# LANL-Bioinformatics/PCRamp

Measured on AMD Instinct MI355X. Metric: primer-pair x target amplification evals/sec, higher is better.
Workload: dtype u32

## Files before the change

pcramp_amd/csrc/pcr_device.hip:

```cpp
#include <hip/hip_runtime.h>
#include <cstring>
#include <rocprim/device/device_radix_sort.hpp>

#include <stdint.h>
#include <string.h>
#include <math.h>
#include <stdlib.h>
#include <string>
#include <vector>
#include <chrono>
#include <algorithm>
#include <unordered_map>
#include <type_traits>
#include <thread>
#include <mutex>
#include <condition_variable>
#include <functional>
#include <memory>
#include <atomic>
#include <cassert>
#include <sched.h>
#include <pthread.h>

#include "../../include/pcramp_hip.h"
// ... 133 lines not shown
		cgh = hi.y | hi.z;
	}
	uint32_t out = 0;
	for(uint32_t j = 0;j < 32;++j){
		if(funnel(nzl, nzh, j) != 0xFFFFFFFFu) continue;
		const uint32_t ngc = __popc(funnel(cgl, cgh, j));
		if(!((gc_ok >> ngc) & 1ull)) continue;
		const uint32_t n2 = __popc(funnel(d2l, d2h, j));
		const uint32_t n3 = __popc(funnel(d3l, d3h, j));
		const uint32_t n4 = __popc(funnel(d4l, d4h, j));
		const uint32_t e = n2 + 2*n4;
		bool exceeds;
		if(e >= 33){ exceeds = true; }
		else{
			uint64_t p3 = 1;
			for(uint32_t k = 0;k < n3;++k) p3 *= 3;
			exceeds = p3 > ((uint64_t)max_degen >> e);
		}
		if(!exceeds) out |= (1u << j);
	}
	valid[gb] = out;
}

struct HitSink { uint32_t *best; Hit *hits; uint32_t *seq_count; uint32_t *counters; uint32_t cap; uint32_t ncand; uint32_t epoch; };

__device__ __forceinline__ void record_hit_inline(const HitSink &k, uint32_t seq, uint32_t cand, uint64_t key, uint32_t cnt)
{
	const uint32_t tagged = (k.epoch << 8) | cnt;
	const uint32_t old = atomicMax(&k.best[(size_t)seq*k.ncand + cand], tagged);
	if(tagged >= old){
		const uint32_t slot = atomicAdd(&k.seq_count[seq], 1u);
		if(slot < k.cap){
			Hit h; h.key = key; h.cand = cand; h.cnt = cnt;
			k.hits[(size_t)seq*k.cap + slot] = h;
		}
		else{ atomicOr(&k.counters[0], 1u); atomicMax(&k.counters[2], slot + 1); }
	}
}

__device__ __noinline__ void record_hit(const HitSink k, uint32_t seq, uint32_t cand, uint64_t key, uint32_t cnt)
{
	record_hit_inline(k, seq, cand, key, cnt);
}

__device__ __forceinline__ uint64_t make_key(uint32_t seq, int32_t loc, uint32_t strand , uint32_t kind, uint32_t ord)
{
	return ((uint64_t)seq << KEY_SEQ_SHIFT) | ((uint64_t)(uint32_t)(loc + LOC_BIAS) << KEY_LOC_SHIFT) |
// ... 411 lines not shown
	Stream stream;
	Stream aux_stream;
	std::string design_text;
	DevBuf<uint64_t> split_where;
	pcr_params params;
	pcrhost::PackFilter filt;
	SeqSet sets[PCR_N_SETS];
	DevBuf<uint32_t> best, counters, mask, status;
	int scan_version = 3;
	bool force_seed1 = false;
	struct S2Key { uint32_t a, c, g, t, floor_; bool operator==(const S2Key &o) const { return a == o.a && c == o.c && g == o.g && t == o.t && floor_ == o.floor_; } };
	struct S2KeyHash { size_t operator()(const S2Key &k) const { uint64_t h = 0x9E3779B97F4A7C15ull; for(uint32_t v : {k.a, k.c, k.g, k.t, k.floor_}){ h ^= v; h *= 0x100000001B3ull; h ^= h >> 29; } return (size_t)h; } };
	struct S2Entry { std::vector<uint32_t> seeds;  uint32_t off_mask; bool seedable; uint4 mask;  };
	std::unordered_map<S2Key, S2Entry, S2KeyHash> s2_cache;
	std::vector<pcrhost::Seed> s2_tmp;
	static constexpr int S3_CHUNK_SETS = 4;
	struct S3Chunks { uint64_t gen = 0; uint32_t total = 0; std::vector<uint32_t> run; };
	struct S3Entry : S2Entry { std::vector<uint8_t> spans;  S3Chunks chunks[S3_CHUNK_SETS]; uint32_t next_slot = 0; };
	std::unordered_map<S2Key, S3Entry, S2KeyHash> s3_cache;
	std::vector<pcrhost::FoldSeed> s3_tmp;
	struct S3Launch { Seed3Slices W; uint32_t n_chunks, per_wg, slice_cap, n_irr_wg; };
	bool no_seed3 = false, s3_attr_set = false;
	bool s3_next = true;
	bool s2_attr_set = false; uint32_t s2_dbg = 0; bool no_irr_index = false;
	std::unordered_map<S2Key, S2Entry, S2KeyHash> s1_cache;
	DevBuf<uint32_t> s1_image, s1_heads, s1_multi, s1_part;
	bool host_seed_tables = false;
	DevBuf<Hit> hits;
	DevBuf<uint64_t> bits_fr, bits_rf;
	DevBuf<OligoDev> oligos;
	DevBuf<SwJob> sw_jobs; DevBuf<SwOut> sw_out; DevBuf<uint8_t> sw_q, sw_qlen, sw_t, entry_codes, entry_lens;
	DevBuf<AmpRec> amp_recs, amp_recs2; DevBuf<BgPairDev> bg_pairs;
	DevBuf<uint64_t> amp_keys; DevBuf<uint32_t> amp_pkeys, amp_pair_start; DevBuf<uint8_t> sort_tmp;
	DevBuf<thermo::Job> th_jobs; DevBuf<thermo::JobOut> th_out; DevBuf<int> th_dg; DevBuf<uint2> th_map; DevBuf<uint32_t> th_bad;
	float th_dg_salt = -1.0f;
	DevBuf<unsigned long long> th_dbg; bool th_attr_set = false;
	std::vector<thermo::Job> th_host_jobs; std::vector<thermo::JobOut> th_host_res;
	MappedBuf<uint8_t> sw_pin; Event sw_done[2];
	DevBuf<pcr_amplicon> mx_amp;
	DevBuf<OligoDev> opt_oligos; DevBuf<uint2> opt_jobs; DevBuf<float> opt_cov; DevBuf<uint32_t> opt_loc, opt_tasks;
	DevBuf<Planes> mx_keys; uint32_t mx_n_keys = 0; DevBuf<uint32_t> mx_count;
	DevBuf<uint8_t> pool_in, pool_tmp; DevBuf<uint32_t> pool_cnt, pool_ord; DevBuf<uint64_t> pool_eoff, pool_ioff, pool_keys; DevBuf<uint2> pool_items; DevBuf<pcr_product> pool_rec;
	DevBuf<uint8_t> site_in, site_tmp; DevBuf<uint32_t> site_cnt, site_ord, site_flag; DevBuf<uint64_t> site_eoff, site_joff, site_keys; DevBuf<uint2> site_items; DevBuf<float4> site_res; DevBuf<pcr_site> site_rec;
	bool site_attr_set = false;
	pcr_comm *shard_comm = nullptr; uint64_t shard_first = 0, shard_n_total = 0; int shard_mode = 0;
	DevBuf<uint64_t> sh_rec, sh_full; DevBuf<uint8_t> sh_stage;
	std::vector<uint64_t> shard_bounds; DevBuf<uint64_t> d_shard_bounds;
	bool design_ready = false; DevBuf<uint64_t> sh_bits;
	std::vector<std::vector<uint8_t> > samp_packed; std::vector<uint64_t> samp_len;
	void drop_shard(){ shard_comm = nullptr; shard_mode = 0; shard_bounds.clear(); design_ready = false; samp_packed.clear(); samp_len.clear(); }
	pcr_comm *trial_comm = nullptr;
// ... 619 lines not shown
	if(hipGetDeviceProperties(&prop, device) != hipSuccess){ g_err = "pcr_create: hipGetDeviceProperties failed"; return nullptr; }
	if(std::string(prop.gcnArchName).find("gfx950") == std::string::npos){
		g_err = std::string("pcr_create: device is ") + prop.gcnArchName + ", this build targets gfx950 only";
		return nullptr;
	}
	pcr_ctx *ctx = new pcr_ctx();
	ctx->device = device;
	if(hip_stream) ctx->stream.borrow((hipStream_t)hip_stream);
	else if(ctx->stream.create() != hipSuccess){ g_err = "pcr_create: hipStreamCreate failed"; delete ctx; return nullptr; }
	if(params){ ctx->params = *params; }
	else{ ctx->params.pack_max_degen = 256; ctx->params.pack_min_gc = 0.0f; ctx->params.pack_max_gc = 1.0f; }
	{ hipDeviceProp_t prop; if(hipGetDeviceProperties(&prop, device) == hipSuccess && prop.multiProcessorCount > 0) ctx->n_cu = (uint32_t)prop.multiProcessorCount; }
	if(const char *v = getenv("PCRAMP_TIMING")) ctx->timing = v[0] == '1';
	ctx->debug_log = getenv("PCRAMP_DEBUG") != nullptr;
	if(const char *v = getenv("PCRAMP_DEBUG_EPOCH")) ctx->debug_epoch = (uint32_t)strtoul(v, nullptr, 0);
	if(const char *v = getenv("PCRAMP_OPT_PM")) ctx->opt_pm_global = v[0] == 'g';
	if(const char *v = getenv("PCRAMP_DEBUG_OPT_TASKS")){ unsigned a = 0, b = 0; if(sscanf(v, "%u,%u", &a, &b) >= 1){ ctx->opt_dbg_wg_tasks = a; ctx->opt_dbg_task_cap = b; } }
	if(const char *v = getenv("PCRAMP_SEED")) ctx->force_seed1 = v[0] == '1';
	if(const char *v = getenv("PCRAMP_SEED_TABLES")) ctx->host_seed_tables = v[0] == 'h';
	if(const char *v = getenv("PCRAMP_S2DBG")) ctx->s2_dbg = (uint32_t)atoi(v);
	if(const char *v = getenv("PCRAMP_IRR_INDEX")) ctx->no_irr_index = v[0] == '0';
	if(const char *v = getenv("PCRAMP_SEED3")) ctx->no_seed3 = v[0] == '0';
	if(const char *v = getenv("PCRAMP_S3_NEXT")) ctx->s3_next = v[0] != '0';
	if(const char *v = getenv("PCRAMP_LAUNCH_THREAD")) ctx->launch_thread = v[0] != '0';
	if(const char *v = getenv("PCRAMP_SCAN")){ if(v[0] == '1') ctx->scan_version = 1; else if(v[0] == '2') ctx->scan_version = 2; }
	{
		const char *v = getenv("PCRAMP_STAGE");
		if(!(v && v[0] == 'k') && prop.isLargeBar){
			DevBuf<uint32_t> probe(true); MappedBuf<uint32_t> back; const std::string err_before = g_err;
			constexpr uint32_t PROBE_WORDS = 1024;
			if(probe.ensure(PROBE_WORDS) == PCR_OK && back.ensure(PROBE_WORDS*sizeof(uint32_t)) == PCR_OK){
				hipPointerAttribute_t at;
				bool ok = hipPointerGetAttributes(&at, probe.p) == hipSuccess;
				for(int round = 0;ok && round < 2;++round){
					volatile uint32_t *w = (volatile uint32_t *)probe.p;
					for(uint32_t i = 0;i < PROBE_WORDS;++i){ w[i] = 0x9E3779B9u*(i + 1) + (uint32_t)round; back.host[i] = 0; }
					__builtin_ia32_sfence();
					hipLaunchKernelGGL(k_stage, dim3(1), dim3(256), 0, ctx->stream, (const uint4 *)probe.p, (uint4 *)back.dev, PROBE_WORDS/4,
						(uint4 *)nullptr, 0u, (uint4 *)nullptr, 0u, (uint4 *)nullptr, 0u);
					ok = hipGetLastError() == hipSuccess && hipStreamSynchronize(ctx->stream) == hipSuccess;
					for(uint32_t i = 0;ok && i < PROBE_WORDS;++i) ok = back.host[i] == 0x9E3779B9u*(i + 1) + (uint32_t)round;
				}
				ctx->direct_ok = ok;
			}
			else{ (void)hipGetLastError(); g_err = err_before; }
		}
// ... 624 lines not shown
```

pcramp_amd/csrc/pcr_host.hpp:

```cpp
#ifndef PCR_HOST_HPP
#define PCR_HOST_HPP

#include <stdint.h>
#include <algorithm>
#include <deque>
#include <vector>

namespace pcrhost {

struct Planes {
	uint32_t a, c, g, t;
};

inline uint32_t bitrev32(uint32_t v)
{
	v = ((v >> 1) & 0x55555555u) | ((v & 0x55555555u) << 1);
	v = ((v >> 2) & 0x33333333u) | ((v & 0x33333333u) << 2);
	v = ((v >> 4) & 0x0F0F0F0Fu) | ((v & 0x0F0F0F0Fu) << 4);
	v = ((v >> 8) & 0x00FF00FFu) | ((v & 0x00FF00FFu) << 8);
	return (v >> 16) | (v << 16);
}

inline unsigned word_get(const uint64_t w[2], int k) { return (unsigned)(w[k >> 4] >> ((15 - (k & 15))*4)) & 0xF; }

// ... 24 lines not shown
	p.c = gather_every_4th(r[0] >> 1) | (gather_every_4th(r[1] >> 1) << 16);
	p.g = gather_every_4th(r[0] >> 2) | (gather_every_4th(r[1] >> 2) << 16);
	p.t = gather_every_4th(r[0] >> 3) | (gather_every_4th(r[1] >> 3) << 16);
	return p;
}

inline void word_of_planes(const Planes &p, uint64_t w[2])
{
	w[0] = w[1] = 0;
	for(int k = 0;k < 32;++k){
		const unsigned v = ((p.a >> k) & 1) | (((p.c >> k) & 1) << 1) | (((p.g >> k) & 1) << 2) | (((p.t >> k) & 1) << 3);
		word_set(w, k, v);
	}
}

inline Planes planes_revcomp(const Planes &p)
{
	Planes r;
	r.a = bitrev32(p.t);
	r.t = bitrev32(p.a);
	r.c = bitrev32(p.g);
	r.g = bitrev32(p.c);
	return r;
}

inline uint32_t planes_occupied(const Planes &p) { return p.a | p.c | p.g | p.t; }
inline int planes_size(const Planes &p) { return __builtin_popcount(planes_occupied(p)); }
inline int planes_start(const Planes &p) { const uint32_t o = planes_occupied(p); return o ? __builtin_ctz(o) : 32; }
inline int planes_stop(const Planes &p) { const uint32_t o = planes_occupied(p); return o ? 31 - __builtin_clz(o) : -1; }

inline unsigned planes_nibble(const Planes &p, int k)
{
	return ((p.a >> k) & 1) | (((p.c >> k) & 1) << 1) | (((p.g >> k) & 1) << 2) | (((p.t >> k) & 1) << 3);
}

inline Planes planes_shift_left(const Planes &p) { Planes r = {p.a >> 1, p.c >> 1, p.g >> 1, p.t >> 1}; return r; }
inline Planes planes_shift_right(const Planes &p) { Planes r = {p.a << 1, p.c << 1, p.g << 1, p.t << 1}; return r; }

struct PackFilter {
	uint32_t max_degen;
	uint64_t gc_ok;
	bool gc_on;

	void set_gc(float min_gc, float max_gc)
	{
		gc_on = (min_gc > 0.0f) || (max_gc < 1.0f);
// ... 658 lines not shown
```

pcramp_amd/csrc/pcr_scan_seed3.inc:

```

constexpr uint32_t PIX_CODES = 1u << 18;
constexpr uint32_t PIX_KEYS = PIX_CODES << 2;
constexpr uint32_t S3_BATCH = 8;

template<bool SCATTER>
__global__ void k_pix_build(const uint32_t *__restrict__ tb, const uint32_t *__restrict__ blk_seq, const uint64_t *__restrict__ blk_off,
	const uint64_t *__restrict__ len, uint64_t total_blocks, uint32_t *__restrict__ count_or_cursor, uint4 *__restrict__ ent)
{
	const uint64_t b = (uint64_t)blockIdx.x*blockDim.x + threadIdx.x;
	if(b >= total_blocks) return;
	const uint32_t seq = blk_seq[b];
	const int64_t p0 = (int64_t)(b - blk_off[seq])*32, L = (int64_t)len[seq];
	uint32_t w[8];
#pragma unroll
	for(int k = 0;k < 8;++k) w[k] = tb[(int64_t)2*(int64_t)b - 2 + k];
#pragma unroll
	for(int i = 0;i < 32;++i){
		if(p0 + i + 9 > L) break;
		const uint32_t ten = (i < 16) ? funnel(w[2], w[3], 2*i) : funnel(w[3], w[4], 2*(i - 16));
		const uint32_t code = ((ten & S2_CODE_MASK) << 2) | ((ten >> 18) & 3u);
		if(SCATTER){
			const uint32_t at = atomicAdd(&count_or_cursor[code], 1u);
			const int jl = (i + 9) >> 4, sl = 2*((i + 9) & 15);
			const int jr = (i + 41) >> 4, sr = 2*((i + 41) & 15);
// ... 53 lines not shown
		const uint32_t sdv = (lane < 16u && i < T3.n_seeds) ? T3.seeds[i] : S2_END;
		const uint32_t orient = T3.or_base + (sdv & 0x1FFu);
		uint32_t first = 0, cnt = 0;
		if(sdv != S2_END && !(orient & 1u)){
			const uint32_t key = (((sdv >> 9) & 31u) << 18) | (sdv >> 14);
			first = IA.ix_first[key]; cnt = IA.ix_last[key] - first;
		}
		const uint32_t incl = s2_scan(cnt);
		const uint32_t total = s2_rl(incl, 63);
		for(uint32_t t0 = 0;t0 < total;t0 += 64u){
			const uint32_t t = t0 + lane;
			uint32_t lo = 0;
#pragma unroll
			for(uint32_t stp = 32u;stp;stp >>= 1){ if((uint32_t)__shfl((int)incl, (int)(lo + stp - 1u)) <= t) lo += stp; }
			const int sl = (int)min(lo, 63u);
			const uint32_t s_incl = (uint32_t)__shfl((int)incl, sl), s_cnt = (uint32_t)__shfl((int)cnt, sl), s_first = (uint32_t)__shfl((int)first, sl);
			const uint32_t c = (uint32_t)__shfl((int)orient, sl) >> 1;
			if(t >= total) continue;
			const IrrDev e = IA.irr[IA.ix_words[s_first + (t - (s_incl - s_cnt))]];
			if(((e.meta >> 8) & 0xFFu) < IA.min_cws || !Q.active[e.seq]) continue;
			const uint32_t n = match_count(e.w.a, e.w.c, e.w.g, e.w.t, cand_fwd[c]);
			if(n >= cand_floor[c]) record_hit(sink, e.seq, c, make_key(e.seq, e.loc, e.meta & 0xFF, 1, (e.meta >> 16) & 0xFF), n);
		}
	}
}

template<uint32_t S3_THREADS>
__global__ __launch_bounds__(S3_THREADS) __attribute__((amdgpu_waves_per_eu(8, 8))) void k_seed3(Seed3Tables T3, Seed3Set Q, IrrArgs2 IA, const uint4 *__restrict__ cand_fwd, const uint32_t *__restrict__ cand_floor,
	HitSink sink, S2Clear Z, Seed3Slices W)
{
	extern __shared__ uint4 s3_dyn[];
	uint4 *const masks = s3_dyn;
	uint32_t *const prefix = (uint32_t *)(masks + T3.n_or);
	uint32_t *const seeds = prefix + T3.slice_cap;
	uint8_t *const floors = (uint8_t *)(seeds + T3.slice_cap);
	uint8_t *const spans = floors + ((T3.n_or + 15u) & ~15u);
	const uint32_t wave = threadIdx.x >> 6, lane = threadIdx.x & 63u;
	for(uint32_t i = blockIdx.x*S3_THREADS + threadIdx.x;i < Z.n0;i += gridDim.x*S3_THREADS) Z.z0[i] = make_uint4(0, 0, 0, 0);
	for(uint32_t i = blockIdx.x*S3_THREADS + threadIdx.x;i < Z.n1;i += gridDim.x*S3_THREADS) Z.z1[i] = make_uint4(0, 0, 0, 0);
	if(Z.ctrl && blockIdx.x == 0 && threadIdx.x == 0){ Z.ctrl[1] = 0; Z.ctrl[3] = 0; }
	for(uint32_t i = threadIdx.x;i < T3.n_or;i += S3_THREADS){ masks[i] = T3.masks[i]; floors[i] = T3.floors[i]; }
	constexpr uint32_t S3_WAVES = S3_THREADS/64;
	if(blockIdx.x < T3.n_irr_wg){
		if(IA.ix_first) s3_irregular(T3, Q, IA, cand_fwd, cand_floor, sink, blockIdx.x*S3_WAVES + wave, T3.n_irr_wg*S3_WAVES, lane);
		return;
	}
// ... 10 lines not shown
			const uint32_t q = q0 + lane*S3_WAVES;
			if(lane < S3_BATCH && q < q_hi){
				uint32_t lo = 0, hi = n_slice - 1u;
				while(hi - lo > 1u){ const uint32_t mid = (lo + hi) >> 1; if(prefix[mid] <= q) lo = mid; else hi = mid; }
				c_sd = seeds[lo];
				const uint32_t key = (c_sd >> 14) << 2, sp = spans[lo];
				const uint32_t f = T3.pix_first[key + (sp & 3u)], e = T3.pix_last[key + (sp >> 2)], j0 = (q - prefix[lo])*64u;
				c_first = f + j0; c_cnt = (e - f) - j0;
			}
		}
		uint4 en[S3_BATCH];
#pragma unroll
		for(int b = 0;b < (int)S3_BATCH;++b){
			const uint32_t first = s2_rl(c_first, b), cnt = s2_rl(c_cnt, b);
			en[b] = make_uint4(0xFFFFFFFFu, 0, 0, 0);
			if(lane < cnt) en[b] = T3.pix_ent[first + lane];
		}
		uint32_t cnt_b[S3_BATCH], g[S3_BATCH]; bool pass_b[S3_BATCH];
#pragma unroll
		for(int b = 0;b < (int)S3_BATCH;++b){
			const uint32_t sdv = s2_rl(c_sd, b);
			const uint32_t off = (sdv >> 9) & 31u, local = sdv & 0x1FFu, code = sdv >> 14;
			g[b] = en[b].x;
			const uint32_t r_lo = funnel(en[b].z, en[b].w, 14);
			const uint4 cx = make_uint4(en[b].y << 2, (funnel(en[b].y, en[b].z, 30) & 0xFFFFu) | (code << 16), (code >> 16) | (r_lo << 2), en[b].w >> 12);
			const uint32_t in = 24u - off, sh = 2u*(in & 15u);
			const uint32_t a0 = (in < 16u) ? funnel(cx.x, cx.y, sh) : funnel(cx.y, cx.z, sh);
			const uint32_t a1 = (in < 16u) ? funnel(cx.y, cx.z, sh) : funnel(cx.z, cx.w, sh);
			cnt_b[b] = (uint32_t)__popc(s2_mux(a0, a1, masks[local]));
			pass_b[b] = g[b] != 0xFFFFFFFFu && cnt_b[b] >= floors[local] && g[b] >= off;
		}
		uint32_t vw[S3_BATCH], info[S3_BATCH], bl[S3_BATCH];
#pragma unroll
		for(int b = 0;b < (int)S3_BATCH;++b){
			vw[b] = 0; info[b] = 0; bl[b] = 0;
			if(pass_b[b]){
				const uint32_t ws = g[b] - ((s2_rl(c_sd, b) >> 9) & 31u);
				vw[b] = Q.valid[ws >> 5]; info[b] = Q.blk_info[ws >> 5]; bl[b] = Q.blk_local[ws >> 5];
			}
		}
#pragma unroll
		for(int b = 0;b < (int)S3_BATCH;++b){
			if(!pass_b[b]) continue;
			const uint32_t sdv = s2_rl(c_sd, b);
			const uint32_t ws = g[b] - ((sdv >> 9) & 31u), seq = info[b] & BLK_SEQ_MASK;
			if(!((vw[b] >> (ws & 31u)) & 1u) || (info[b] & (BLK_DEGEN | BLK_INACTIVE))) continue;
			const uint32_t p_local = bl[b]*32u + (ws & 31u);
			const uint32_t orient = T3.or_base + (sdv & 0x1FFu), c = orient >> 1;
			if(orient & 1u) record_hit(sink, seq, c, make_key(seq, (int32_t)p_local + 31, 2, 0, 0), cnt_b[b]);
			else record_hit(sink, seq, c, make_key(seq, (int32_t)p_local, 1, 0, 0), cnt_b[b]);
		}
	}
	if(IA.ix_first && T3.n_irr_wg == 0) s3_irregular(T3, Q, IA, cand_fwd, cand_floor, sink, gw, n_gw, lane);
}
```

pcramp_amd/csrc/pcr_screen.inc:

```
__device__ __forceinline__ bool db_slot(uint32_t g, uint32_t n, uint32_t cap, const uint32_t *__restrict__ touched,
	const uint32_t *__restrict__ seg_hi, uint32_t &slot)
{
	if(g >= n) return false;
	const uint32_t seq = touched[g/cap];
	slot = seq*cap + g % cap;
	return slot < seg_hi[seq];
}

constexpr int MATCH_WAVES = 4;
__global__ __launch_bounds__(64*MATCH_WAVES) void k_match(const DevEntry *__restrict__ db, uint32_t n_touched, const uint32_t *__restrict__ n_touched_dev, uint32_t cap,
	const uint32_t *__restrict__ touched, const uint32_t *__restrict__ seg_hi, const OligoDev *__restrict__ oligos, uint32_t n_oligo,
	uint32_t mask_words, uint32_t *__restrict__ mask, uint32_t *__restrict__ status,
	const uint32_t *__restrict__ pub_counters, PassMail *pub_mail, uint32_t pub_seq)
{
	if(blockIdx.x == 0 && threadIdx.x == 0 && status) status[0] = 0;
	if(pub_mail && blockIdx.x == 0 && threadIdx.x < 64){
		if(threadIdx.x < 4) pub_mail->counters[threadIdx.x] = pub_counters[threadIdx.x];
		__threadfence_system();
		__builtin_amdgcn_wave_barrier();
		if(threadIdx.x == 0) __hip_atomic_store((uint32_t *)&pub_mail->seq, pub_seq, __ATOMIC_RELEASE, __HIP_MEMORY_SCOPE_SYSTEM);
	}
	if(n_touched_dev) n_touched = *n_touched_dev;
	const uint32_t lane = threadIdx.x & 63u, sub = lane >> 5, ol = lane & 31u;
	for(uint32_t t_idx = blockIdx.x*MATCH_WAVES + (threadIdx.x >> 6);t_idx < n_touched;t_idx += gridDim.x*MATCH_WAVES){
// ... 254 lines not shown
			if(eos && has_split(planes, blk_base, amp_start, amp_len)) continue;
			best = fmaxf(best, r.id);
		}
		if(best < 0.0f) continue;
		uint64_t *dst = (orient == 0) ? bits_fr : bits_rf;
		const uint64_t bit = 1ull << (seq & 63);
		for(uint32_t v = 0;v < n_variants;++v){
			const float var = identity(variants[v], ee.w, use_taq);
			const float f = (side == 0) ? var : best, r2 = (side == 0) ? best : var;
			if(sqrtf(__fmul_rn(f, r2)) >= ident_thr)
				atomicOr((unsigned long long *)&dst[(size_t)v*bit_words + (seq >> 6)], bit);
		}
	}
}

constexpr uint32_t POST_CAP = 64, POST_MASK_WORDS = 4;
struct PostEnt { Planes w; int32_t loc; uint32_t strand; };
template<int POST_WAVES>
struct PostShared {
	OligoDev ol[32*POST_MASK_WORDS];
	uint64_t keys[POST_WAVES][POST_CAP]; PostEnt ent[POST_WAVES][POST_CAP]; uint32_t msk[POST_WAVES][POST_CAP][POST_MASK_WORDS];
};

template<int POST_WAVES>
__global__ __launch_bounds__(64*POST_WAVES) void k_post(const Hit *__restrict__ hits, uint32_t *__restrict__ seq_count,
	const uint32_t *__restrict__ best, uint32_t ncand, const uint4 *__restrict__ planes, const uint64_t *__restrict__ blk_off,
	const IrrDev *__restrict__ irr, const uint32_t *__restrict__ irr_off, DevEntry *__restrict__ db, uint32_t *__restrict__ seg_hi,
	uint32_t *__restrict__ counters, uint32_t epoch, uint32_t n_seq,
	const OligoDev *__restrict__ oligos, uint32_t n_pairs, uint32_t mask_words,
	const uint64_t *__restrict__ len, const uint8_t *__restrict__ active, int32_t amp_min, int32_t amp_max, float ident_thr, int use_taq,
	uint64_t *__restrict__ bits_fr, uint64_t *__restrict__ bits_rf, uint64_t bit_words, PassMail *pub_mail, uint32_t pub_seq)
{
	__shared__ PostShared<POST_WAVES> sh;
	const uint32_t wave = threadIdx.x >> 6, lane = threadIdx.x & 63u;
	if(pub_mail && blockIdx.x == 0 && wave == 0){
		if(lane < 4) pub_mail->counters[lane] = (lane == 3) ? N_TOUCHED_UNKNOWN_DEV : counters[lane];
		__threadfence_system();
		__builtin_amdgcn_wave_barrier();
		if(lane == 0) __hip_atomic_store((uint32_t *)&pub_mail->seq, pub_seq, __ATOMIC_RELEASE, __HIP_MEMORY_SCOPE_SYSTEM);
	}
	if(blockIdx.x == 0 && wave == 0 && lane < 4) counters[lane] = 0;
	const uint32_t seq = blockIdx.x*POST_WAVES + wave;
	const uint32_t n_raw = (seq < n_seq) ? seq_count[seq] : 0u;
	const uint32_t n = min(n_raw, POST_CAP);
	if(seq < n_seq && lane == 0){
		if(n_raw) seq_count[seq] = 0;
		else seg_hi[seq] = 0;
	}
	const uint32_t seq_c = min(seq, n_seq - 1u);
	const uint64_t base = blk_off[seq_c];
	const int32_t L = (int32_t)len[seq_c];
	const uint32_t is_active = active[seq_c];
	if(__syncthreads_or((int)n)){
		const uint32_t nw = 2*n_pairs*(uint32_t)(sizeof(OligoDev)/4);
		for(uint32_t i = threadIdx.x;i < nw;i += 64*POST_WAVES) ((uint32_t *)sh.ol)[i] = ((const uint32_t *)oligos)[i];
		__syncthreads();
	}
	if(n == 0) return;
	uint64_t *keys = sh.keys[wave];
	PostEnt *ent = sh.ent[wave];
	uint64_t k = ~0ull;
	if(lane < n){
		const Hit h = hits[(size_t)seq*POST_CAP + lane];
		if(((epoch << 8) | h.cnt) == best[(size_t)seq*ncand + h.cand]) k = h.key;
	}
	keys[lane] = k;
	wave_sync();
	uint32_t np2 = 1; while(np2 < n) np2 <<= 1;
	for(uint32_t kk = 2;kk <= np2;kk <<= 1){
		for(uint32_t j = kk >> 1;j > 0;j >>= 1){
			const uint32_t l = lane ^ j;
			if(l > lane && l < np2){
				const uint64_t a = keys[lane], b = keys[l];
				const bool up = ((lane & kk) == 0);
				if((a > b) == up){ keys[lane] = b; keys[l] = a; }
			}
			wave_sync();
		}
	}
	k = keys[lane];
	const bool distinct = k != ~0ull && (lane == 0 || keys[lane - 1] != k);
	const uint64_t dmask = __ballot(distinct);
	const uint32_t run = (uint32_t)__builtin_popcountll(dmask);
	const uint32_t rank = (uint32_t)__builtin_popcountll(dmask & ((1ull << lane) - 1ull));
	if(lane == 0) seg_hi[seq] = seq*POST_CAP + run;
	if(distinct){
		DevEntry e;
		materialise_entry_at(k, planes, base, irr, irr_off, e);
		db[(size_t)seq*POST_CAP + rank] = e;
		PostEnt pe; pe.w = e.w; pe.loc = e.loc; pe.strand = e.strand;
		ent[rank] = pe;
	}
	wave_sync();
	if(n_pairs == 0) return;
	const uint32_t n_oligo = 2*n_pairs;
	PostEnt me; me.w.a = me.w.c = me.w.g = me.w.t = 0; me.loc = 0; me.strand = 0;
	if(lane < run) me = ent[lane];
	for(uint32_t g = 0;2*g < mask_words;++g){
		const uint32_t o = g*64 + lane;
		Planes m; m.a = m.c = m.g = m.t = 0; uint32_t fl = 0xFFFFFFFFu;
		if(o < n_oligo){ m = sh.ol[o].m; fl = sh.ol[o].floor2; }
		for(uint32_t e = 0;e < run;++e){
			const Planes w = ent[e].w;
			const uint32_t cnt = __popc((w.a & m.a) | (w.c & m.c) | (w.g & m.g) | (w.t & m.t));
			const uint64_t bal = __ballot(cnt >= fl);
			if(lane == 0){
				sh.msk[wave][e][2*g] = (uint32_t)bal;
				if(2*g + 1 < mask_words) sh.msk[wave][e][2*g + 1] = (uint32_t)(bal >> 32);
			}
		}
	}
// ... 184 lines not shown
```

pcramp_amd/csrc/pcr_select.inc:

```
namespace {

struct PlanLists {
	std::vector<uint32_t> s2_seeds; std::vector<uint4> s2_masks; std::vector<uint8_t> s2_floors;
	std::vector<uint32_t> s2_group_end, s2_group_offmask, s2_group_or, s2_group_nor;
	std::vector<pcr_ctx::S3Launch> s3_launch;
	std::vector<uint32_t> s3_prefix;
	std::vector<uint8_t> s3_spans;
	std::vector<uint32_t> s1_seeds;
	void clear()
	{
		s2_seeds.clear(); s2_masks.clear(); s2_floors.clear(); s2_group_end.clear(); s2_group_offmask.clear(); s2_group_or.clear(); s2_group_nor.clear();
		s3_launch.clear(); s3_prefix.clear(); s3_spans.clear(); s1_seeds.clear();
	}
};

inline uint32_t spread16(uint32_t v)
{
	v &= 0xFFFFu;
	v = (v | (v << 8)) & 0x00FF00FFu; v = (v | (v << 4)) & 0x0F0F0F0Fu;
	v = (v | (v << 2)) & 0x33333333u; return (v | (v << 1)) & 0x55555555u;
}

constexpr uint32_t S2_MAX_GROUPS = 4096;
bool plan_seed2(pcr_ctx *ctx, PlanLists &L, const std::vector<pcrhost::Candidate> &cand, std::vector<uint32_t> &or_seed, std::vector<uint32_t> &or_plain, uint32_t &irr_off_mask,
// ... 660 lines not shown
}

int launch_scans(pcr_ctx *ctx, SeqSet &S, const ScanPlan &P, const PlanLists &L, const StagedTables &T, const FusedAmp *fa, const HitSink &sink)
{
	int rc = PCR_OK;
	const uint32_t ncand = sink.ncand;
	if(S.n_tiles){
		ProfScope scan_prof(ctx, PCR_PROF_SCAN, ctx->prof && (ctx->prof_pass++ % ctx->prof_stride) == 0);
		if(P.need_plain && (rc = launch_scan2(ctx, S, T.plain.T, ncand, sink, T.plain.d_tab, T.plain.d_bias, nullptr, S.n_tiles, T.plain.d_map)) != PCR_OK) return rc;
		if(P.form == ScanForm::Popcount) rc = launch_popcount(ctx, S, sink);
		else if(is_seed1(P.form)) rc = launch_seed1(ctx, S, P, T, sink);
		else if(is_seed2(P.form)) rc = launch_seed_groups(ctx, S, P, L, T, fa, sink);
		if(rc != PCR_OK) return rc;
		if(P.need_seedset && (rc = launch_scan2(ctx, S, T.seedset.T, ncand, sink, T.seedset.d_tab, T.seedset.d_bias, S.degen_tiles.p, S.n_degen_tiles,
			T.seedset.d_map)) != PCR_OK) return rc;
		scan_prof.finish();
	}
	const bool irr_taken = S.n_tiles && (is_seed1(P.form) || is_seed2(P.form));
	if(P.n_live && !irr_taken) rc = launch_irregular(ctx, S, P, sink);
	return rc;
}


template<class K>
void launch_post(K kernel, uint32_t waves, pcr_ctx *ctx, SeqSet &S, const HitSink &sink, const FusedAmp *fa, uint32_t seq)
{
	hipLaunchKernelGGL(kernel, dim3((S.n + waves - 1)/waves), dim3(64*waves), 0, ctx->stream, sink.hits, sink.seq_count, sink.best, sink.ncand, S.planes.p,
		S.d_blk_off.p, S.irr.p, S.irr_off.p, S.db.p, S.d_seg_hi, sink.counters, sink.epoch, S.n,
		fa->d_oligos, fa->n_pairs, (2*fa->n_pairs + 31)/32, S.d_len.p, S.d_active.p, fa->a->amp_min, fa->a->amp_max,
		fa->a->ident_threshold, fa->a->use_taq_mama, fa->d_fr, fa->d_rf, (uint64_t)((S.n + 63)/64), ctx->mail.dev + (seq % pcr_ctx::MAIL_RING), seq);
}
int fused_tail(pcr_ctx *ctx, SeqSet &S, const HitSink &sink, FusedAmp *fa, uint32_t reserved_seq)
{
	const uint32_t seq = reserved_seq ? reserved_seq : ++ctx->mail_seq;
	if(sink.cap == POST_CAP){
		launch_post(k_post<8>, 8, ctx, S, sink, fa, seq);
		S.ctrl_clean = true; S.touched_from_seg = true;
	}
	else if(sink.cap == 128) launch_post(k_post_big<128, 4>, 4, ctx, S, sink, fa, seq);
	else launch_post(k_post_big<256, 4>, 4, ctx, S, sink, fa, seq);
	HIP_TRY(hipGetLastError());
	fa->posted = true;
	S.touched_built = false;
	return PCR_OK;
}

template<class K, class... Extra>
void launch_finalize(K kernel, dim3 grid, dim3 block, size_t lds, pcr_ctx *ctx, SeqSet &S, const HitSink &sink, Extra... extra)
{
	hipLaunchKernelGGL(kernel, grid, block, lds, ctx->stream, sink.hits, sink.seq_count, sink.cap, sink.best, sink.ncand, S.planes.p, S.d_blk_off.p, S.irr.p,
		S.irr_off.p, S.db.p, S.d_seg_hi, sink.counters, sink.epoch, S.touched.p, extra...);
}
template<bool ALL = false>
int plain_tail(pcr_ctx *ctx, SeqSet &S, const HitSink &sink, bool async, FusedAmp *fa)
{
	int rc;
	hipLaunchKernelGGL(k_touched, dim3((S.n + 255)/256), dim3(256), 0, ctx->stream, sink.seq_count, S.n, sink.counters, S.touched.p);
	HIP_TRY(hipGetLastError());
	S.touched_built = true;
// ... 8 lines not shown
	++ctx->mail_seq;
	if(async && fa && fa->staged){ fa->pub_seq = ctx->mail_seq; fa->pub_counters = sink.counters; }
	else{
		hipLaunchKernelGGL(k_publish, dim3(1), dim3(64), 0, ctx->stream, sink.counters, ctx->mail.dev + (ctx->mail_seq % pcr_ctx::MAIL_RING), ctx->mail_seq);
		HIP_TRY(hipGetLastError());
	}
	return PCR_OK;
}

uint32_t resized_buckets(bool overflowed, uint32_t cap, uint32_t largest_fill, int attempt)
{
	if(overflowed){
		uint32_t want = cap*2;
		while(want < largest_fill && want < MAX_BUCKET_CAP_GLOBAL) want *= 2;
		return want;
	}
	if(cap <= 64 || attempt >= 12) return 0;
	uint32_t want = 64;
	while(want < largest_fill + largest_fill/16) want *= 2;
	return (want*4 <= cap) ? want : 0;
}

inline bool fused_tail_fits(uint32_t cap, uint32_t n_pairs) { return (cap == POST_CAP || cap == 128 || cap == 256) && 2*n_pairs <= 32*POST_MASK_WORDS; }
inline bool buckets_fit(uint64_t n_slots) { return n_slots < (uint64_t(1) << 32) && n_slots*(sizeof(Hit) + sizeof(DevEntry)) <= (uint64_t(96) << 30); }

inline bool begin_pass(SeqSet &S)
{
	S.have_db = false; S.n_entries = 0;
	const bool ctrl_was_clean = S.ctrl_clean;
	S.ctrl_clean = false; S.touched_from_seg = false;
	return ctrl_was_clean;
}

int plan_pass(pcr_ctx *ctx, PassJob &J, const pcr_pair *pairs, uint32_t n_pairs)
{
	SeqSet &S = ctx->sets[J.which];
	HostTimer timer(ctx, 0);
	if(ctx->timing) ++ctx->n_timed;
	pcrhost::build_candidates((const uint64_t *)pairs, n_pairs, J.opt5 != 0, J.opt3 != 0, J.thr, J.cand);
	const uint32_t ncand = (uint32_t)J.cand.size();
	if(S.n == 0 || ncand == 0) return PCR_OK;
	int rc;
	if((rc = choose_scan_form(ctx, S, J.cand, J.opt5, J.opt3, J.min_len, J.P, J.L)) != PCR_OK) return rc;
	if(ctx->debug_log) fprintf(stderr, "[pcramp] scan plan: form=%s, %u candidates, %zu seeded orientations (%zu seeds), %zu plain, %u/%u IUPAC tiles, %u-slot buckets\n",
		form_name(J.P.form), ncand, J.P.or_seed.size(), J.P.n_seeds, J.P.or_plain.size(), S.n_degen_tiles, S.n_tiles, S.bucket_cap);
	prepare_tables(S, J, J.has_fa ? &J.fa : nullptr);
// ... 28 lines not shown
	HostTimer timer(ctx, 1);
	int rc;
	if((rc = ctx->best.ensure((size_t)S.n*ncand)) != PCR_OK) return rc;
	if(ctx->best.generation != ctx->best_seen){
		HIP_TRY(hipMemsetAsync(ctx->best.p, 0, ctx->best.cap*sizeof(uint32_t), ctx->stream));
		ctx->best_seen = ctx->best.generation; ctx->epoch = std::min(ctx->debug_epoch, EPOCH_LIMIT);
	}
	StagedTables T;
	if((rc = stage_tables(ctx, S, J, fa, async, ctrl_was_clean, T)) != PCR_OK) return rc;

	timer.next(2);
	uint32_t h_counters[4];
	if((rc = S.touched.ensure(S.n)) != PCR_OK) return rc;
	S.d_seg_hi = S.ctrl.p + 8 + S.n;
	for(int attempt = 0;;++attempt){
		const uint32_t cap = S.bucket_cap;
		const uint64_t n_slots = (uint64_t)S.n*cap;
		if(!buckets_fit(n_slots)){
			assert(J.seq == 0);
			S.bucket_cap = 64;
			g_err = "pcr_select_words: the per-sequence hit buckets would not fit (too many tied sites per sequence)"; return PCR_ERR_CAPACITY;
		}
		if((rc = ctx->hits.ensure(n_slots)) != PCR_OK) return rc;
		if((rc = S.db.ensure(n_slots)) != PCR_OK) return rc;
		if(attempt > 0) HIP_TRY(hipMemsetAsync(S.ctrl.p, 0, (8 + 2*(size_t)S.n)*sizeof(uint32_t), ctx->stream));
		if(ctx->epoch >= EPOCH_LIMIT){
			HIP_TRY(hipMemsetAsync(ctx->best.p, 0, ctx->best.cap*sizeof(uint32_t), ctx->stream));
			ctx->epoch = 0;
		}
		++ctx->epoch;
		HitSink sink; sink.best = ctx->best.p; sink.hits = ctx->hits.p; sink.seq_count = S.ctrl.p + 8;
		sink.counters = S.ctrl.p; sink.cap = cap; sink.ncand = ncand; sink.epoch = ctx->epoch;
		const bool fused = async && fa && fa->staged && fused_tail_fits(cap, fa->n_pairs);
		if(J.seq && !fused){ g_err = "pcr_screen_device: a pipelined pass lost its fused tail"; return PCR_ERR_STATE; }
		if((rc = launch_scans(ctx, S, P, J.L, T, fa, sink)) != PCR_OK) return rc;
		if((rc = fused ? fused_tail(ctx, S, sink, fa, J.seq) : plain_tail(ctx, S, sink, async, fa)) != PCR_OK) return rc;
		if(async){
			S.db_cap = cap; S.n_slots = n_slots;
			S.n_touched = N_TOUCHED_UNKNOWN; S.n_entries = 1; S.have_db = true;
			return PCR_OK;
		}
		timer.next(3);
		if((rc = mail_wait(ctx, ctx->mail_seq, h_counters)) != PCR_OK) return rc;
		timer.next(2);
		S.db_cap = cap; S.n_slots = n_slots;
		const bool overflowed = (h_counters[0] & 1u) != 0;
		if(overflowed && (attempt >= 12 || cap >= MAX_BUCKET_CAP_GLOBAL)){ g_err = "pcr_select_words: more than 65536 candidate sites in one sequence (per-sequence bucket limit)"; return PCR_ERR_CAPACITY; }
		const uint32_t want = resized_buckets(overflowed, cap, h_counters[2], attempt);
		if(!want) break;
		S.bucket_cap = want;
	}
	if(ctx->debug_log) fprintf(stderr, "[pcramp] pass done: %u-slot buckets, largest fill %u, %u sequences with entries\n", S.db_cap, h_counters[2], h_counters[3]);
	S.n_touched = h_counters[3];
	S.n_entries = S.n_touched ? 1 : 0;
	S.have_db = true;
	if(n_entries_out){
		if((rc = count_entries(ctx, S)) != PCR_OK) return rc;
		*n_entries_out = S.n_entries;
	}
// ... 235 lines not shown
```

pcramp_amd/csrc/pcr_select_sites.inc:

```

namespace {

struct SitesSlow { const uint4 *cand_fwd, *cand_rc; const uint32_t *cand_floor; uint32_t ncand; uint32_t pad; };

__device__ __noinline__ uint32_t sites_recount(uint32_t bits, uint32_t o_base, uint32_t have, uint32_t wa, uint32_t wc, uint32_t wg, uint32_t wt,
	const SitesSlow *A)
{
	if(have & 1u) bits &= 0xAAAAAAAAu;
	if(have & 2u) bits &= 0x55555555u;
	const uint32_t ncand = A->ncand;
	while(bits){
		const uint32_t j = __ffs(bits) - 1;
		bits &= bits - 1;
		const uint32_t o = o_base + j, c = o >> 1;
		if(c >= ncand) continue;
		const uint32_t cnt = match_count(wa, wc, wg, wt, (o & 1u) ? A->cand_rc[c] : A->cand_fwd[c]);
		if(cnt >= A->cand_floor[c]){
			have |= 1u << (o & 1u);
			bits &= (o & 1u) ? 0x55555555u : 0xAAAAAAAAu;
		}
	}
	return have;
}

// ... 200 lines not shown
	for(uint32_t o = 0;o < 2*ncand;++o) P.or_plain[o] = o;
	if(ctx->debug_log) fprintf(stderr, "[pcramp] all-sites plan: %u candidates, %u/%u IUPAC tiles, %u live irregular words, %u-slot buckets\n",
		ncand, S.n_degen_tiles, S.n_tiles, P.n_live, S.bucket_cap);
	StagedTables T;
	prepare_tables(S, J, nullptr);
	timer.next(1);
	if((rc = stage_tables(ctx, S, J, nullptr, false, false, T)) != PCR_OK) return rc;

	timer.next(2);
	uint32_t h_counters[4];
	if((rc = S.touched.ensure(S.n)) != PCR_OK) return rc;
	S.d_seg_hi = S.ctrl.p + 8 + S.n;
	for(int attempt = 0;;++attempt){
		const uint32_t cap = S.bucket_cap;
		const uint64_t n_slots = (uint64_t)S.n*cap;
		if(n_slots >= (uint64_t(1) << 32) || n_slots*(sizeof(Hit) + sizeof(DevEntry)) > (uint64_t(96) << 30)){
			S.bucket_cap = 64;
			g_err = "pcr_select_sites: the per-sequence hit buckets would not fit (too many sites per sequence)"; return PCR_ERR_CAPACITY;
		}
		if((rc = ctx->hits.ensure(n_slots)) != PCR_OK) return rc;
		if((rc = S.db.ensure(n_slots)) != PCR_OK) return rc;
		if(attempt > 0) HIP_TRY(hipMemsetAsync(S.ctrl.p, 0, (8 + 2*(size_t)S.n)*sizeof(uint32_t), ctx->stream));
		HitSink sink; sink.best = nullptr; sink.hits = ctx->hits.p; sink.seq_count = S.ctrl.p + 8;
		sink.counters = S.ctrl.p; sink.cap = cap; sink.ncand = ncand; sink.epoch = 0;
		if((rc = launch_sites(ctx, S, P, T.plain, sink)) != PCR_OK) return rc;
		if((rc = plain_tail<true>(ctx, S, sink, false, nullptr)) != PCR_OK) return rc;
		timer.next(3);
		if((rc = mail_wait(ctx, ctx->mail_seq, h_counters)) != PCR_OK) return rc;
		timer.next(2);
		S.db_cap = cap; S.n_slots = n_slots;
		const bool overflowed = (h_counters[0] & 1u) != 0;
		if(overflowed && (attempt >= 12 || cap >= MAX_BUCKET_CAP_GLOBAL)){
			S.bucket_cap = 64;
			g_err = "pcr_select_sites: more than 65536 candidate sites in one sequence (per-sequence bucket limit)"; return PCR_ERR_CAPACITY;
		}
		const uint32_t want = resized_buckets(overflowed, cap, h_counters[2], attempt);
		if(!want) break;
		S.bucket_cap = want;
	}
	if(ctx->debug_log) fprintf(stderr, "[pcramp] all-sites pass done: %u-slot buckets, largest fill %u, %u sequences with entries\n", S.db_cap, h_counters[2], h_counters[3]);
	S.n_touched = h_counters[3];
	S.n_entries = S.n_touched ? 1 : 0;
	S.have_db = true;
	if(n_entries_out){
		if((rc = count_entries(ctx, S)) != PCR_OK) return rc;
		*n_entries_out = S.n_entries;
	}
// ... 16 lines not shown
```

Baseline: 23.64 billion.

## Record hit windows in seed3 scan and skip per-candidate best lookup in post

The seed3 scan now writes each hit's 64-bit window code next to the hit record. The fused k_post tail then rebuilds the entry planes from that code, so it no longer re-materialises them from sequence blocks. Within a wave, k_post resolves the per-candidate maximum with readlane instead of reading the global best array. This removes scattered global reads from the post kernel. In exchange it adds an extra buffer write per hit and an O(n) lane loop, and the scan's hit loop is split into two passes.

New measurement: 23.47 billion, median of 2. No clear change (-0.7%).

```diff
diff --git a/pcramp_amd/csrc/pcr_device.hip b/pcramp_amd/csrc/pcr_device.hip
--- a/pcramp_amd/csrc/pcr_device.hip
+++ b/pcramp_amd/csrc/pcr_device.hip
@@ -179,7 +179,7 @@
 	valid[gb] = out;
 }
 
-struct HitSink { uint32_t *best; Hit *hits; uint32_t *seq_count; uint32_t *counters; uint32_t cap; uint32_t ncand; uint32_t epoch; };
+struct HitSink { uint32_t *best; Hit *hits; uint32_t *seq_count; uint32_t *counters; uint32_t cap; uint32_t ncand; uint32_t epoch; uint2 *wins; };
 
 __device__ __forceinline__ void record_hit_inline(const HitSink &k, uint32_t seq, uint32_t cand, uint64_t key, uint32_t cnt)
 {
@@ -637,11 +637,13 @@
 	struct S3Launch { Seed3Slices W; uint32_t n_chunks, per_wg, slice_cap, n_irr_wg; };
 	bool no_seed3 = false, s3_attr_set = false;
 	bool s3_next = true;
+	bool post_inline = true;
 	bool s2_attr_set = false; uint32_t s2_dbg = 0; bool no_irr_index = false;
 	std::unordered_map<S2Key, S2Entry, S2KeyHash> s1_cache;
 	DevBuf<uint32_t> s1_image, s1_heads, s1_multi, s1_part;
 	bool host_seed_tables = false;
 	DevBuf<Hit> hits;
+	DevBuf<uint2> wins;
 	DevBuf<uint64_t> bits_fr, bits_rf;
 	DevBuf<OligoDev> oligos;
 	DevBuf<SwJob> sw_jobs; DevBuf<SwOut> sw_out; DevBuf<uint8_t> sw_q, sw_qlen, sw_t, entry_codes, entry_lens;
@@ -1307,6 +1309,7 @@
 	if(const char *v = getenv("PCRAMP_IRR_INDEX")) ctx->no_irr_index = v[0] == '0';
 	if(const char *v = getenv("PCRAMP_SEED3")) ctx->no_seed3 = v[0] == '0';
 	if(const char *v = getenv("PCRAMP_S3_NEXT")) ctx->s3_next = v[0] != '0';
+	if(const char *v = getenv("PCRAMP_POST_INLINE")) ctx->post_inline = v[0] != '0';
 	if(const char *v = getenv("PCRAMP_LAUNCH_THREAD")) ctx->launch_thread = v[0] != '0';
 	if(const char *v = getenv("PCRAMP_SCAN")){ if(v[0] == '1') ctx->scan_version = 1; else if(v[0] == '2') ctx->scan_version = 2; }
 	{
diff --git a/pcramp_amd/csrc/pcr_host.hpp b/pcramp_amd/csrc/pcr_host.hpp
--- a/pcramp_amd/csrc/pcr_host.hpp
+++ b/pcramp_amd/csrc/pcr_host.hpp
@@ -70,6 +70,39 @@
 	r.c = bitrev32(p.g);
 	r.g = bitrev32(p.c);
 	return r;
+}
+
+#if defined(__HIPCC__)
+#define PCR_HOST_DEVICE __host__ __device__
+#else
+#define PCR_HOST_DEVICE
+#endif
+PCR_HOST_DEVICE inline uint32_t gather_even_bits(uint64_t x)
+{
+	x &= 0x5555555555555555ull;
+	x = (x | (x >> 1)) & 0x3333333333333333ull;
+	x = (x | (x >> 2)) & 0x0F0F0F0F0F0F0F0Full;
+	x = (x | (x >> 4)) & 0x00FF00FF00FF00FFull;
+	x = (x | (x >> 8)) & 0x0000FFFF0000FFFFull;
+	return (uint32_t)(x | (x >> 16));
+}
+PCR_HOST_DEVICE inline uint32_t bitrev32_hd(uint32_t v)
+{
+#if defined(__HIP_DEVICE_COMPILE__)
+	return __builtin_bitreverse32(v);
+#else
+	return bitrev32(v);
+#endif
+}
+PCR_HOST_DEVICE inline Planes planes_of_window_codes(uint32_t w0, uint32_t w1, uint32_t strand )
+{
+	const uint64_t code = (uint64_t)w0 | ((uint64_t)w1 << 32);
+	const uint32_t lo = gather_even_bits(code), hi = gather_even_bits(code >> 1);
+	const uint32_t a = ~lo & ~hi, c = lo & ~hi, g = ~lo & hi, t = lo & hi;
+	Planes p;
+	if(strand == 1){ p.a = a; p.c = c; p.g = g; p.t = t; }
+	else{ p.a = bitrev32_hd(t); p.t = bitrev32_hd(a); p.c = bitrev32_hd(g); p.g = bitrev32_hd(c); }
+	return p;
 }
 
 inline uint32_t planes_occupied(const Planes &p) { return p.a | p.c | p.g | p.t; }
diff --git a/pcramp_amd/csrc/pcr_scan_seed3.inc b/pcramp_amd/csrc/pcr_scan_seed3.inc
--- a/pcramp_amd/csrc/pcr_scan_seed3.inc
+++ b/pcramp_amd/csrc/pcr_scan_seed3.inc
@@ -99,6 +99,34 @@
 			const uint32_t n = match_count(e.w.a, e.w.c, e.w.g, e.w.t, cand_fwd[c]);
 			if(n >= cand_floor[c]) record_hit(sink, e.seq, c, make_key(e.seq, e.loc, e.meta & 0xFF, 1, (e.meta >> 16) & 0xFF), n);
 		}
+	}
+}
+
+__device__ __forceinline__ void s3_window(const uint4 en, uint32_t off, uint32_t code, uint32_t &a0, uint32_t &a1)
+{
+	const uint32_t r_lo = funnel(en.z, en.w, 14);
+	const uint4 cx = make_uint4(en.y << 2, (funnel(en.y, en.z, 30) & 0xFFFFu) | (code << 16), (code >> 16) | (r_lo << 2), en.w >> 12);
+	const uint32_t in = 24u - off, sh = 2u*(in & 15u);
+	a0 = (in < 16u) ? funnel(cx.x, cx.y, sh) : funnel(cx.y, cx.z, sh);
+	a1 = (in < 16u) ? funnel(cx.y, cx.z, sh) : funnel(cx.z, cx.w, sh);
+}
+
+__device__ __forceinline__ void record_hit_window(const HitSink k, uint32_t seq, uint32_t cand, uint64_t key, uint32_t cnt, const uint4 *__restrict__ entry, uint32_t sdv)
+{
+	uint4 en = *entry;
+	const uint32_t tagged = (k.epoch << 8) | cnt;
+	const uint32_t old = atomicMax(&k.best[(size_t)seq*k.ncand + cand], tagged);
+	asm volatile("" : "+v"(en.y), "+v"(en.z), "+v"(en.w));
+	if(tagged >= old){
+		const uint32_t slot = atomicAdd(&k.seq_count[seq], 1u);
+		if(slot < k.cap){
+			Hit h; h.key = key; h.cand = cand; h.cnt = cnt;
+			uint32_t a0, a1;
+			s3_window(en, (sdv >> 9) & 31u, sdv >> 14, a0, a1);
+			k.hits[(size_t)seq*k.cap + slot] = h;
+			k.wins[(size_t)seq*k.cap + slot] = make_uint2(a0, a1);
+		}
+		else{ atomicOr(&k.counters[0], 1u); atomicMax(&k.counters[2], slot + 1); }
 	}
 }
 
@@ -155,11 +183,8 @@
 			const uint32_t sdv = s2_rl(c_sd, b);
 			const uint32_t off = (sdv >> 9) & 31u, local = sdv & 0x1FFu, code = sdv >> 14;
 			g[b] = en[b].x;
-			const uint32_t r_lo = funnel(en[b].z, en[b].w, 14);
-			const uint4 cx = make_uint4(en[b].y << 2, (funnel(en[b].y, en[b].z, 30) & 0xFFFFu) | (code << 16), (code >> 16) | (r_lo << 2), en[b].w >> 12);
-			const uint32_t in = 24u - off, sh = 2u*(in & 15u);
-			const uint32_t a0 = (in < 16u) ? funnel(cx.x, cx.y, sh) : funnel(cx.y, cx.z, sh);
-			const uint32_t a1 = (in < 16u) ? funnel(cx.y, cx.z, sh) : funnel(cx.z, cx.w, sh);
+			uint32_t a0, a1;
+			s3_window(en[b], off, code, a0, a1);
 			cnt_b[b] = (uint32_t)__popc(s2_mux(a0, a1, masks[local]));
 			pass_b[b] = g[b] != 0xFFFFFFFFu && cnt_b[b] >= floors[local] && g[b] >= off;
 		}
@@ -174,14 +199,21 @@
 		}
 #pragma unroll
 		for(int b = 0;b < (int)S3_BATCH;++b){
+			asm volatile("" : "+v"(vw[b]), "+v"(info[b]), "+v"(bl[b]));
+			if(!pass_b[b]) continue;
+			const uint32_t ws = g[b] - ((s2_rl(c_sd, b) >> 9) & 31u);
+			pass_b[b] = ((vw[b] >> (ws & 31u)) & 1u) && !(info[b] & (BLK_DEGEN | BLK_INACTIVE));
+			g[b] = bl[b]*32u + (ws & 31u);
+			info[b] &= BLK_SEQ_MASK;
+		}
+#pragma unroll
+		for(int b = 0;b < (int)S3_BATCH;++b){
 			if(!pass_b[b]) continue;
 			const uint32_t sdv = s2_rl(c_sd, b);
-			const uint32_t ws = g[b] - ((sdv >> 9) & 31u), seq = info[b] & BLK_SEQ_MASK;
-			if(!((vw[b] >> (ws & 31u)) & 1u) || (info[b] & (BLK_DEGEN | BLK_INACTIVE))) continue;
-			const uint32_t p_local = bl[b]*32u + (ws & 31u);
+			const uint32_t seq = info[b], p_local = g[b];
 			const uint32_t orient = T3.or_base + (sdv & 0x1FFu), c = orient >> 1;
-			if(orient & 1u) record_hit(sink, seq, c, make_key(seq, (int32_t)p_local + 31, 2, 0, 0), cnt_b[b]);
-			else record_hit(sink, seq, c, make_key(seq, (int32_t)p_local, 1, 0, 0), cnt_b[b]);
+			const uint4 *const entry = T3.pix_ent + (s2_rl(c_first, b) + lane);
+			record_hit_window(sink, seq, c, make_key(seq, (int32_t)p_local + ((orient & 1u) ? 31 : 0), 1u + (orient & 1u), 0, 0), cnt_b[b], entry, sdv);
 		}
 	}
 	if(IA.ix_first && T3.n_irr_wg == 0) s3_irregular(T3, Q, IA, cand_fwd, cand_floor, sink, gw, n_gw, lane);
diff --git a/pcramp_amd/csrc/pcr_screen.inc b/pcramp_amd/csrc/pcr_screen.inc
--- a/pcramp_amd/csrc/pcr_screen.inc
+++ b/pcramp_amd/csrc/pcr_screen.inc
@@ -300,14 +300,15 @@
 	uint64_t keys[POST_WAVES][POST_CAP]; PostEnt ent[POST_WAVES][POST_CAP]; uint32_t msk[POST_WAVES][POST_CAP][POST_MASK_WORDS];
 };
 
-template<int POST_WAVES>
+template<int POST_WAVES, bool INLINE>
 __global__ __launch_bounds__(64*POST_WAVES) void k_post(const Hit *__restrict__ hits, uint32_t *__restrict__ seq_count,
 	const uint32_t *__restrict__ best, uint32_t ncand, const uint4 *__restrict__ planes, const uint64_t *__restrict__ blk_off,
 	const IrrDev *__restrict__ irr, const uint32_t *__restrict__ irr_off, DevEntry *__restrict__ db, uint32_t *__restrict__ seg_hi,
 	uint32_t *__restrict__ counters, uint32_t epoch, uint32_t n_seq,
 	const OligoDev *__restrict__ oligos, uint32_t n_pairs, uint32_t mask_words,
 	const uint64_t *__restrict__ len, const uint8_t *__restrict__ active, int32_t amp_min, int32_t amp_max, float ident_thr, int use_taq,
-	uint64_t *__restrict__ bits_fr, uint64_t *__restrict__ bits_rf, uint64_t bit_words, PassMail *pub_mail, uint32_t pub_seq)
+	uint64_t *__restrict__ bits_fr, uint64_t *__restrict__ bits_rf, uint64_t bit_words, PassMail *pub_mail, uint32_t pub_seq,
+	const uint2 *__restrict__ wins)
 {
 	__shared__ PostShared<POST_WAVES> sh;
 	const uint32_t wave = threadIdx.x >> 6, lane = threadIdx.x & 63u;
@@ -338,9 +339,20 @@
 	uint64_t *keys = sh.keys[wave];
 	PostEnt *ent = sh.ent[wave];
 	uint64_t k = ~0ull;
-	if(lane < n){
-		const Hit h = hits[(size_t)seq*POST_CAP + lane];
-		if(((epoch << 8) | h.cnt) == best[(size_t)seq*ncand + h.cand]) k = h.key;
+	uint2 win = make_uint2(0u, 0u);
+	if(INLINE){
+		Hit h; h.key = 0; h.cand = 0; h.cnt = 0;
+		if(lane < n){ h = hits[(size_t)seq*POST_CAP + lane]; win = wins[(size_t)seq*POST_CAP + lane]; }
+		uint32_t mx = 0;
+		for(uint32_t j = 0;j < n;++j){
+			const uint32_t cj = (uint32_t)__builtin_amdgcn_readlane((int)h.cand, (int)j), nj = (uint32_t)__builtin_amdgcn_readlane((int)h.cnt, (int)j);
+			if(cj == h.cand) mx = max(mx, nj);
+		}
+		if(lane < n && h.cnt == mx) k = (h.key << 6) | lane;
+	}
+	else if(lane < n){
+		const Hit hh = hits[(size_t)seq*POST_CAP + lane];
+		if(((epoch << 8) | hh.cnt) == best[(size_t)seq*ncand + hh.cand]) k = hh.key;
 	}
 	keys[lane] = k;
 	wave_sync();
@@ -357,14 +369,25 @@
 		}
 	}
 	k = keys[lane];
-	const bool distinct = k != ~0ull && (lane == 0 || keys[lane - 1] != k);
+	bool distinct;
+	if(INLINE){
+		distinct = k != ~0ull && (lane == 0 || (keys[lane - 1] >> 6) != (k >> 6));
+		const int src = (int)(k & 63u);
+		win.x = (uint32_t)__shfl((int)win.x, src); win.y = (uint32_t)__shfl((int)win.y, src);
+		k = ((uint64_t)seq << KEY_SEQ_SHIFT) | ((k >> 6) & ((1ull << KEY_SEQ_SHIFT) - 1ull));
+	}
+	else distinct = k != ~0ull && (lane == 0 || keys[lane - 1] != k);
 	const uint64_t dmask = __ballot(distinct);
 	const uint32_t run = (uint32_t)__builtin_popcountll(dmask);
 	const uint32_t rank = (uint32_t)__builtin_popcountll(dmask & ((1ull << lane) - 1ull));
 	if(lane == 0) seg_hi[seq] = seq*POST_CAP + run;
 	if(distinct){
 		DevEntry e;
-		materialise_entry_at(k, planes, base, irr, irr_off, e);
+		if(INLINE && !((k >> 6) & 1ull)){
+			e.loc = (int32_t)(uint32_t)((k >> KEY_LOC_SHIFT) & 0xFFFFFFFFull) - LOC_BIAS; e.seq = seq; e.strand = (uint32_t)((k >> 7) & 1) + 1; e.pad = 0;
+			e.w = pcrhost::planes_of_window_codes(win.x, win.y, e.strand);
+		}
+		else materialise_entry_at(k, planes, base, irr, irr_off, e);
 		db[(size_t)seq*POST_CAP + rank] = e;
 		PostEnt pe; pe.w = e.w; pe.loc = e.loc; pe.strand = e.strand;
 		ent[rank] = pe;
diff --git a/pcramp_amd/csrc/pcr_select.inc b/pcramp_amd/csrc/pcr_select.inc
--- a/pcramp_amd/csrc/pcr_select.inc
+++ b/pcramp_amd/csrc/pcr_select.inc
@@ -706,19 +706,20 @@
 }
 
 
-template<class K>
-void launch_post(K kernel, uint32_t waves, pcr_ctx *ctx, SeqSet &S, const HitSink &sink, const FusedAmp *fa, uint32_t seq)
+template<class K, class... Extra>
+void launch_post(K kernel, uint32_t waves, pcr_ctx *ctx, SeqSet &S, const HitSink &sink, const FusedAmp *fa, uint32_t seq, Extra... extra)
 {
 	hipLaunchKernelGGL(kernel, dim3((S.n + waves - 1)/waves), dim3(64*waves), 0, ctx->stream, sink.hits, sink.seq_count, sink.best, sink.ncand, S.planes.p,
 		S.d_blk_off.p, S.irr.p, S.irr_off.p, S.db.p, S.d_seg_hi, sink.counters, sink.epoch, S.n,
 		fa->d_oligos, fa->n_pairs, (2*fa->n_pairs + 31)/32, S.d_len.p, S.d_active.p, fa->a->amp_min, fa->a->amp_max,
-		fa->a->ident_threshold, fa->a->use_taq_mama, fa->d_fr, fa->d_rf, (uint64_t)((S.n + 63)/64), ctx->mail.dev + (seq % pcr_ctx::MAIL_RING), seq);
-}
-int fused_tail(pcr_ctx *ctx, SeqSet &S, const HitSink &sink, FusedAmp *fa, uint32_t reserved_seq)
+		fa->a->ident_threshold, fa->a->use_taq_mama, fa->d_fr, fa->d_rf, (uint64_t)((S.n + 63)/64), ctx->mail.dev + (seq % pcr_ctx::MAIL_RING), seq, extra...);
+}
+int fused_tail(pcr_ctx *ctx, SeqSet &S, const HitSink &sink, FusedAmp *fa, uint32_t reserved_seq, bool inline_windows)
 {
 	const uint32_t seq = reserved_seq ? reserved_seq : ++ctx->mail_seq;
 	if(sink.cap == POST_CAP){
-		launch_post(k_post<8>, 8, ctx, S, sink, fa, seq);
+		if(inline_windows) launch_post(k_post<8, true>, 8, ctx, S, sink, fa, seq, (const uint2 *)sink.wins);
+		else launch_post(k_post<8, false>, 8, ctx, S, sink, fa, seq, (const uint2 *)nullptr);
 		S.ctrl_clean = true; S.touched_from_seg = true;
 	}
 	else if(sink.cap == 128) launch_post(k_post_big<128, 4>, 4, ctx, S, sink, fa, seq);
@@ -773,6 +774,10 @@
 }
 
 inline bool fused_tail_fits(uint32_t cap, uint32_t n_pairs) { return (cap == POST_CAP || cap == 128 || cap == 256) && 2*n_pairs <= 32*POST_MASK_WORDS; }
+inline bool post_inline_fits(const pcr_ctx *ctx, const ScanPlan &P, uint32_t cap)
+{
+	return ctx->post_inline && P.form == ScanForm::Seed3 && !P.need_plain && !P.need_seedset && cap == POST_CAP;
+}
 inline bool buckets_fit(uint64_t n_slots) { return n_slots < (uint64_t(1) << 32) && n_slots*(sizeof(Hit) + sizeof(DevEntry)) <= (uint64_t(96) << 30); }
 
 inline bool begin_pass(SeqSet &S)
@@ -847,6 +852,7 @@
 			g_err = "pcr_select_words: the per-sequence hit buckets would not fit (too many tied sites per sequence)"; return PCR_ERR_CAPACITY;
 		}
 		if((rc = ctx->hits.ensure(n_slots)) != PCR_OK) return rc;
+		if(P.form == ScanForm::Seed3 && (rc = ctx->wins.ensure(n_slots)) != PCR_OK) return rc;
 		if((rc = S.db.ensure(n_slots)) != PCR_OK) return rc;
 		if(attempt > 0) HIP_TRY(hipMemsetAsync(S.ctrl.p, 0, (8 + 2*(size_t)S.n)*sizeof(uint32_t), ctx->stream));
 		if(ctx->epoch >= EPOCH_LIMIT){
@@ -856,10 +862,13 @@
 		++ctx->epoch;
 		HitSink sink; sink.best = ctx->best.p; sink.hits = ctx->hits.p; sink.seq_count = S.ctrl.p + 8;
 		sink.counters = S.ctrl.p; sink.cap = cap; sink.ncand = ncand; sink.epoch = ctx->epoch;
+		sink.wins = P.form == ScanForm::Seed3 ? ctx->wins.p : nullptr;
 		const bool fused = async && fa && fa->staged && fused_tail_fits(cap, fa->n_pairs);
+		const bool inline_tail = fused && post_inline_fits(ctx, P, cap);
+		if(ctx->debug_log && fused) fprintf(stderr, "[pcramp] staging: tail=%s\n", cap != POST_CAP ? "k_post_big" : inline_tail ? "k_post-inline" : "k_post");
 		if(J.seq && !fused){ g_err = "pcr_screen_device: a pipelined pass lost its fused tail"; return PCR_ERR_STATE; }
 		if((rc = launch_scans(ctx, S, P, J.L, T, fa, sink)) != PCR_OK) return rc;
-		if((rc = fused ? fused_tail(ctx, S, sink, fa, J.seq) : plain_tail(ctx, S, sink, async, fa)) != PCR_OK) return rc;
+		if((rc = fused ? fused_tail(ctx, S, sink, fa, J.seq, inline_tail) : plain_tail(ctx, S, sink, async, fa)) != PCR_OK) return rc;
 		if(async){
 			S.db_cap = cap; S.n_slots = n_slots;
 			S.n_touched = N_TOUCHED_UNKNOWN; S.n_entries = 1; S.have_db = true;
diff --git a/pcramp_amd/csrc/pcr_select_sites.inc b/pcramp_amd/csrc/pcr_select_sites.inc
--- a/pcramp_amd/csrc/pcr_select_sites.inc
+++ b/pcramp_amd/csrc/pcr_select_sites.inc
@@ -246,7 +246,7 @@
 		if((rc = S.db.ensure(n_slots)) != PCR_OK) return rc;
 		if(attempt > 0) HIP_TRY(hipMemsetAsync(S.ctrl.p, 0, (8 + 2*(size_t)S.n)*sizeof(uint32_t), ctx->stream));
 		HitSink sink; sink.best = nullptr; sink.hits = ctx->hits.p; sink.seq_count = S.ctrl.p + 8;
-		sink.counters = S.ctrl.p; sink.cap = cap; sink.ncand = ncand; sink.epoch = 0;
+		sink.counters = S.ctrl.p; sink.cap = cap; sink.ncand = ncand; sink.epoch = 0; sink.wins = nullptr;
 		if((rc = launch_sites(ctx, S, P, T.plain, sink)) != PCR_OK) return rc;
 		if((rc = plain_tail<true>(ctx, S, sink, false, nullptr)) != PCR_OK) return rc;
 		timer.next(3);
```
